# nihalsid/retrieval-fuse

Hardware: AMD Instinct MI355X
Metric: 64^3 TSDF chunks/sec (retrieve+attend+refine) (higher is better)
Workload: dtype f32

## Files before the change

### retrieval-fuse_amd/csrc/build.py

```python
import os
import subprocess
import sys
from concurrent.futures import ThreadPoolExecutor
from pathlib import Path

HERE = Path(__file__).resolve().parent
OUT = HERE.parent / 'rfuse' / 'librfuse_hip.so'
SOURCES = ['capi.hip', 'conv3d.hip', 'conv3d_mfma.hip', 'conv3d_up.hip', 'conv3d_up_split.hip', 'conv3d_split.hip', 'conv3d_split_zc.hip', 'conv3d_e2_split.hip', 'conv3d_small.hip', 'conv3d_backward.hip', 'conv3d_wgrad_split.hip', 'conv_valid_mfma.hip', 'conv_valid_split.hip', 'conv_valid_split_pg.hip', 'conv_valid_backward.hip', 'linear.hip', 'attention.hip', 'attention_backward.hip', 'attention_fused.hip', 'retrieval.hip', 'mesh.hip', 'metrics.hip', 'mesh_metrics.hip', 'shape_loss.hip', 'ntxent.hip', 'iou_matrix.hip']
FLAGS = ['--offload-arch=gfx950', '-O3', '-std=c++17', '-fPIC', '-Wall', '-Wno-unused-function']
EXTRA_FLAGS = {'attention.hip': ['-ffp-contract=off'], 'attention_backward.hip': ['-ffp-contract=off'], 'attention_fused.hip': ['-ffp-contract=off'], 'retrieval.hip': ['-ffp-contract=off'],
               'mesh_metrics.hip': ['-ffp-contract=off'],
               'shape_loss.hip': ['-ffp-contract=off'],
               'ntxent.hip': ['-ffp-contract=off', '-fno-slp-vectorize'],
               'iou_matrix.hip': ['-ffp-contract=off'],
               'conv3d_mfma.hip': ['-fno-slp-vectorize'], 'conv3d_up.hip': ['-fno-slp-vectorize']}


def _hipcc():
    return os.environ.get('HIPCC', '/opt/rocm/bin/hipcc')


def _llvm_bin():
    import shutil
    roots = [Path(os.path.realpath(_hipcc())).parents[1], Path(os.environ.get('ROCM_PATH', '/opt/rocm')), Path('/opt/rocm')]
    for r in roots:
        for sub in ('lib/llvm/bin', 'llvm/bin'):
            if (r / sub / 'llvm-objdump').exists():
                return r / sub
    found = shutil.which('llvm-objdump')
    if found:
        return Path(found).parent
    raise RuntimeError('check_isa: llvm-objdump not found under %s' % ', '.join(str(r) for r in roots))


def _stale(obj, deps):
    return (not obj.exists()) or any(d.stat().st_mtime > obj.stat().st_mtime for d in deps)


def unsafe_packed_fp32(asm_text):
    import re
    bad = []
    for line in asm_text.splitlines():
        m = re.search(r'\bv_pk_(?:fma|mul|add)_f32\b.*?\bop_sel:\[([01,]+)\]', line)
        if m and '1' in m.group(1).split(',')[1:]:
            bad.append(line.strip())
    return bad


def check_isa(so=OUT, name=None):
    import shutil
    import tempfile
    with tempfile.TemporaryDirectory() as tmp:
        lib = Path(tmp) / (name or so.name)
        shutil.copy(so, lib)
        llvm_bin = _llvm_bin()
        subprocess.run([str(llvm_bin / 'llvm-objdump'), '--offloading', str(lib)], check=True, stdout=subprocess.DEVNULL, cwd=tmp)
        cos = sorted(Path(tmp).glob(lib.name + '.*gfx950*'))
        if not cos:
            raise RuntimeError('check_isa: no gfx950 code object found in %s' % so)
        bad = []
        for co in cos:
            asm = subprocess.run([str(llvm_bin / 'llvm-objdump'), '-d', str(co)], check=True, capture_output=True, text=True).stdout
            bad += unsafe_packed_fp32(asm)
    if bad:
        raise RuntimeError('check_isa: %d packed-fp32 instructions with op_sel on src1/src2 (wrong results beside F16 MFMAs on gfx950), e.g.\n  %s'
                           % (len(bad), '\n  '.join(bad[:5])))
    return len(cos)


def build(force=False, verbose=False, out=None, extra_flags=(), objdir=None):
    hipcc = _hipcc()
    OUT = Path(out) if out is not None else globals()['OUT']
    objdir = Path(objdir) if objdir is not None else HERE / 'build'
    objdir.mkdir(exist_ok=True, parents=True)
    headers = [HERE / 'common.h', HERE / 'conv_box.h', HERE / 'conv_split_common.h', HERE / 'conv_split_args.h', HERE / 'split_operand.h', HERE / 'attn_row.h', HERE / 'philox.h',
               HERE.parents[1] / 'include' / 'rfuse.h', HERE.parents[1] / 'include' / 'rfuse_eval.h', HERE.parents[1] / 'include' / 'rfuse_train.h',
               HERE.parents[1] / 'include' / 'rfuse_contrastive.h', HERE.parents[1] / 'include' / 'rfuse_pairs.h', HERE.parents[1] / 'include' / 'rfuse_attn_train.h']

    def compile_one(src):
        obj = objdir / (src.replace('.hip', '.o'))
        if force or _stale(obj, [HERE / src, HERE / 'build.py'] + headers):
            cmd = [hipcc] + FLAGS + list(extra_flags) + EXTRA_FLAGS.get(src, []) + ['-c', str(HERE / src), '-o', str(obj)]
            if verbose:
                print(' '.join(cmd))
            subprocess.run(cmd, check=True)
        return obj

    with ThreadPoolExecutor(max_workers=len(SOURCES)) as ex:
        objs = list(ex.map(compile_one, SOURCES))
    if force or _stale(OUT, objs):
        tmp_out = OUT.with_name(OUT.name + '.unchecked')
        cmd = [hipcc, '--offload-arch=gfx950', '-shared', '-fPIC', '-o', str(tmp_out)] + [str(o) for o in objs]
        if verbose:
            print(' '.join(cmd))
        try:
            subprocess.run(cmd, check=True)
            check_isa(tmp_out, name='librfuse_hip.so')
        except BaseException:
            tmp_out.unlink(missing_ok=True)
            OUT.unlink(missing_ok=True)
            raise
        os.replace(tmp_out, OUT)
    return OUT


TESTKIT_SRC = HERE.parents[1] / 'tests' / 'testkit' / 'testkit.hip'
TESTKIT_OUT = TESTKIT_SRC.parent / 'librfuse_testkit.so'


def build_testkit(force=False):
    if force or _stale(TESTKIT_OUT, [TESTKIT_SRC, HERE / 'build.py']):
        subprocess.run([_hipcc(), '--offload-arch=gfx950', '-O3', '-std=c++17', '-shared', '-fPIC', '-o', str(TESTKIT_OUT), str(TESTKIT_SRC)], check=True)
    return TESTKIT_OUT


if __name__ == '__main__':
    print(build(force='--force' in sys.argv, verbose=True))
    print(build_testkit(force='--force' in sys.argv))
```

### retrieval-fuse_amd/model/unet.py

```python
import math

import torch
from torch import nn

from rfuse import ops, routes


class GroupNormParams(nn.Module):

    def __init__(self, num_groups, num_channels, eps=1e-5):
        super().__init__()
        if num_channels < num_groups:
            num_groups = 1
        assert num_channels % num_groups == 0, \
            f'Expected number of channels in input to be divisible by num_groups. num_channels={num_channels}, num_groups={num_groups}'
        self.num_groups, self.num_channels, self.eps = num_groups, num_channels, eps
        self.weight = nn.Parameter(torch.ones(num_channels))
        self.bias = nn.Parameter(torch.zeros(num_channels))

    def extra_repr(self):
        return f'{self.num_groups}, {self.num_channels}, eps={self.eps}'


class Conv3dParams(nn.Module):
# ... 131 lines not shown
            n, edge, pre = x.n, x.edge, ops.conv3d_split_pre_presplit(x, c1.conv.packed_split(), cmid, *second).data
        else:
            n, ch0, _, edge = ops._src_dims(x, upsampled)
            if route in ('cin1_presplit', 'cin1_presplit_handed'):
                pre = ops.conv3d_cin1_presplit(x, g1.weight, g1.bias, g1.eps, c1.conv.packed(), cmid, *second)
            else:
                aff = ops.gn_affine(x, upsampled, g1.weight, g1.bias, g1.num_groups, g1.eps)
                if route == 'box_presplit':
                    pre = ops.conv3d_split_presplit(x, aff, c1.conv.packed_split(), cmid, *second)
                else:
                    pre = ops.conv3d_up_split_presplit(x, upsampled, aff, c1.conv.packed_up_split(ch0), cmid, *second, parity_major=pm)
        if route == 'cin1_presplit_handed':
            ng = next_block.SingleConv1.groupnorm
            return ops.conv3d_split_pre_relu_pool_presplit(pre, cmid, n, edge, c2.conv.packed_split(), cout, ng.weight, ng.bias, ng.num_groups, ng.eps)
        return ops.conv3d_split_pre_relu(pre, cmid, n, edge, c2.conv.packed_split(), cout, pool=pool, parity_major=pm)


class DoubleConv(_ConvPair):

    def __init__(self, in_channels, out_channels, encoder, kernel_size=3, order='gcr', num_groups=8):
        super().__init__()
        if encoder:
            c1_in, c1_out = in_channels, max(out_channels // 2, in_channels)
            c2_in, c2_out = c1_out, out_channels
        else:
            c1_in, c1_out = in_channels, out_channels
            c2_in, c2_out = out_channels, out_channels
        self.SingleConv1 = SingleConv(c1_in, c1_out, kernel_size, order, num_groups)
        self.SingleConv2 = SingleConv(c2_in, c2_out, kernel_size, order, num_groups)


class StepDownDoubleConv(_ConvPair):
    ENCODER_FORMS = False

    def __init__(self, in_channels, out_channels, encoder, kernel_size=3, order='gcr', num_groups=8):
        super().__init__()
        self.encoder = encoder
        mid = (in_channels + out_channels) // 2
        self.SingleConv1 = SingleConv(in_channels, mid, kernel_size, order, num_groups)
        self.SingleConv2 = SingleConv(mid, out_channels, kernel_size, order, num_groups)


class Encoder(nn.Module):

    def __init__(self, in_channels, out_channels, conv_kernel_size=3, apply_pooling=True, pool_kernel_size=(2, 2, 2),
                 pool_type='max', basic_module=DoubleConv, conv_layer_order='gcr', num_groups=8):
        super().__init__()
        if apply_pooling and (pool_type != 'max' or tuple(pool_kernel_size) != (2, 2, 2)):
            raise NotImplementedError('only MaxPool3d(2) is built')
        self.apply_pooling = apply_pooling
        self.basic_module = basic_module(in_channels, out_channels, encoder=True, kernel_size=conv_kernel_size,
                                         order=conv_layer_order, num_groups=num_groups)

    def forward(self, x, prepooled=None, pool=None, next_block=None):
        if self.apply_pooling:
            if prepooled is not None:
                x = prepooled
            elif ops.needs_grad(x):
                x = torch.nn.functional.max_pool3d(x, 2)
            else:
                x = ops.maxpool2(x)
        return self.basic_module(x, pool=pool, next_block=next_block)


class Decoder(nn.Module):

    def __init__(self, in_channels, out_channels, kernel_size=3, scale_factor=(2, 2, 2), basic_module=DoubleConv,
                 conv_layer_order='gcr', num_groups=8, mode='nearest'):
        super().__init__()
        if basic_module not in (DoubleConv, StepDownDoubleConv) or mode != 'nearest' or tuple(scale_factor) != (2, 2, 2):
            raise NotImplementedError('only nearest x2 upsampling with concat joining is built')
        self.basic_module = basic_module(in_channels, out_channels, encoder=False, kernel_size=kernel_size,
                                         order=conv_layer_order, num_groups=num_groups)

    def forward(self, encoder_features, x):
        if encoder_features.shape[2] != 2 * x.shape[2]:
            raise NotImplementedError('skip connection must be exactly twice the decoder input resolution')
        return self.basic_module(encoder_features, x)


class DecoderNoJoining(Decoder):

    def forward(self, x):
        return self.basic_module(None, x)


def number_of_features_per_level(init_channel_number, num_levels):
    return [init_channel_number * 2 ** k for k in range(num_levels)]


class UNet3D(nn.Module):

    def __init__(self, in_channels, out_channels, final_sigmoid=True, f_maps=64, layer_order='gcr', num_groups=8, num_levels=4,
                 is_segmentation=True, remove_n_final_layers=0, final_conv=False, **kwargs):
        super().__init__()
        if final_conv or is_segmentation:
            raise NotImplementedError('final_conv / segmentation heads are never instantiated by the refinement path')
        if isinstance(f_maps, int):
            f_maps = number_of_features_per_level(f_maps, num_levels=num_levels)
        encoders = []
        for i, out_feature_num in enumerate(f_maps):
            encoders.append(Encoder(in_channels if i == 0 else f_maps[i - 1], out_feature_num, apply_pooling=(i > 0),
                                    basic_module=DoubleConv, conv_layer_order=layer_order, num_groups=num_groups))
        self.encoders = nn.ModuleList(encoders)

        reversed_f_maps = list(reversed(f_maps))
        if remove_n_final_layers > 0:
            reversed_f_maps = reversed_f_maps[:-remove_n_final_layers]
        outs = list(reversed_f_maps)
        outs[-1] = out_channels
        decoders = []
        for i in range(len(reversed_f_maps) - 1):
            in_feature_num = reversed_f_maps[i] + reversed_f_maps[i + 1]
            last_and_trimmed = i == (len(reversed_f_maps) - 2) and remove_n_final_layers > 0
            decoders.append(Decoder(in_feature_num, outs[i + 1], basic_module=StepDownDoubleConv if last_and_trimmed else DoubleConv,
                                    conv_layer_order=layer_order, num_groups=num_groups))
        self.decoders = nn.ModuleList(decoders)

    def forward(self, x, after_encoders=None):
        feats = []
        n_enc, n_dec = len(self.encoders), len(self.decoders)
        pooled = None
        for i, encoder in enumerate(self.encoders):
            if i == n_enc - 1:
                x, pooled = encoder(x, prepooled=pooled), None
            else:
                is_skip = i >= n_enc - 1 - n_dec
                nxt = self.encoders[i + 1].basic_module
                x, pooled = encoder(x, prepooled=pooled, pool='also' if is_skip else 'only', next_block=nxt if isinstance(nxt, DoubleConv) else None)
            feats.insert(0, x)
        feats = feats[1:]
        if after_encoders is not None:
            after_encoders()
        for decoder, skip in zip(self.decoders, feats):
            x = decoder(skip, x)
        return x
```

### retrieval-fuse_amd/rfuse/_lib.py

```python
import ctypes
import os
import re
from pathlib import Path

import torch

_HERE = Path(__file__).resolve().parent
LIB_PATH = Path(os.environ.get('RFUSE_LIB', _HERE / 'librfuse_hip.so'))
HEADER_PATH = _HERE.parents[1] / 'include' / 'rfuse.h'
EVAL_HEADER_PATH = _HERE.parents[1] / 'include' / 'rfuse_eval.h'
TRAIN_HEADER_PATH = _HERE.parents[1] / 'include' / 'rfuse_train.h'
CONTRASTIVE_HEADER_PATH = _HERE.parents[1] / 'include' / 'rfuse_contrastive.h'
PAIRS_HEADER_PATH = _HERE.parents[1] / 'include' / 'rfuse_pairs.h'
ATTN_TRAIN_HEADER_PATH = _HERE.parents[1] / 'include' / 'rfuse_attn_train.h'

_SCALARS = {'int': ctypes.c_int, 'float': ctypes.c_float, 'size_t': ctypes.c_size_t, 'int64_t': ctypes.c_int64, 'long long': ctypes.c_int64}


def parse_header(text):
    text = re.sub(r'/\*.*?\*/', ' ', text, flags=re.S)
    text = re.sub(r'^[ \t]*#.*$', ' ', text, flags=re.M)
    text = re.sub(r'extern\s+"C"\s*\{|\}', ' ', text)

    def where(chunk):
        m = re.search(r'(\w+)\s*\(', chunk)
        return '%s: %r' % (m.group(1) if m else '?', ' '.join(chunk.split()))

    *decls, rest = text.split(';')
    if rest.strip():
        raise ValueError('declaration without its `;` -- %s' % where(rest))

    def ctype(decl, fn, restype=False):
        decl = ' '.join(decl.replace('*', ' * ').split())
        if restype and decl == 'const char *':
            return ctypes.c_char_p
        if decl.endswith('*'):
            return ctypes.c_void_p
        if decl not in _SCALARS:
            raise ValueError('%s: type %r is outside the vocabulary of the binding (%s, pointers)' % (fn, decl, ', '.join(_SCALARS)))
        return _SCALARS[decl]

    table = {}
    for decl in decls:
        m = re.fullmatch(r'\s*([\w\s*]+?)\b(\w+)\s*\(([\w\s*,]*)\)\s*', decl)
        if m is None:
            raise ValueError('cannot read the declaration of %s' % where(decl))
        ret, fn, params = m.groups()
        params = [] if params.strip() == 'void' else [re.fullmatch(r'\s*(\w[\w\s*]*[\s*])(\w+)\s*', q) for q in params.split(',')]
        if None in params:
            raise ValueError('%s: every parameter needs a type and a name' % fn)
        table[fn] = (ctype(ret, fn, True), [ctype(q.group(1), fn) for q in params], [q.group(2) for q in params])
    return table


SIGNATURES = parse_header(HEADER_PATH.read_text())
EVAL_SIGNATURES = parse_header(EVAL_HEADER_PATH.read_text())
TRAIN_SIGNATURES = parse_header(TRAIN_HEADER_PATH.read_text())
CONTRASTIVE_SIGNATURES = parse_header(CONTRASTIVE_HEADER_PATH.read_text())
PAIRS_SIGNATURES = parse_header(PAIRS_HEADER_PATH.read_text())
ATTN_TRAIN_SIGNATURES = parse_header(ATTN_TRAIN_HEADER_PATH.read_text())


def is_status(name, table=None):
    res, _, params = (SIGNATURES if table is None else table)[name]
    return res is ctypes.c_int and params[-1:] == ['stream']


def _raise_on_status(rc, fn, args):
    if rc != 0:
        check(rc, fn.__name__)
    return rc


_lib = None
_eval = None
_train = None
_contrastive = None
_pairs = None
_attn_train = None


class _Library:

    def __init__(self, cdll, table=SIGNATURES):
        self._cdll = cdll
        self._table = table
        self._direct = {}
        for name, (res, args, _) in table.items():
            fn = getattr(cdll, name)
            fn.restype = res
            fn.argtypes = args
            if is_status(name, table):
                fn.errcheck = _raise_on_status
            self._direct[name] = fn
            setattr(self, name, fn)

    def start_profile(self, records, only=None):
        def timed(name, fn):
            def call(*args):
                e0, e1 = torch.cuda.Event(enable_timing=True), torch.cuda.Event(enable_timing=True)
                e0.record()
                rc = fn(*args)
                e1.record()
                records.append((name, tuple(a for a in args if isinstance(a, int)), e0, e1, tuple(i for i, a in enumerate(args) if a is None or (isinstance(a, ctypes.c_void_p) and not a.value))))
                return rc
            return call
        for name, (res, args, _) in self._table.items():
            if only is not None and name not in only:
                continue
            if res is ctypes.c_int and args:
                setattr(self, name, timed(name, self._direct[name]))

    def stop_profile(self):
        for name, fn in self._direct.items():
            setattr(self, name, fn)


def load():
    global _lib
    if _lib is not None:
        return _lib
    if not LIB_PATH.exists():
        raise RuntimeError(
            'librfuse_hip.so not found at %s -- build it with `python retrieval-fuse_amd/csrc/build.py` '
            '(or __graft_entry__.build()).  There is no CPU fallback for the refinement hot path.' % LIB_PATH)
    _lib = _Library(ctypes.CDLL(str(LIB_PATH)))
    return _lib


def load_eval():
    global _eval
    if _eval is None:
        _eval = _Library(load()._cdll, EVAL_SIGNATURES)
    return _eval


def load_train():
    global _train
    if _train is None:
        _train = _Library(load()._cdll, TRAIN_SIGNATURES)
    return _train


def load_contrastive():
    global _contrastive
    if _contrastive is None:
        _contrastive = _Library(load()._cdll, CONTRASTIVE_SIGNATURES)
    return _contrastive


def load_pairs():
    global _pairs
    if _pairs is None:
        _pairs = _Library(load()._cdll, PAIRS_SIGNATURES)
    return _pairs


def load_attn_train():
    global _attn_train
    if _attn_train is None:
        _attn_train = _Library(load()._cdll, ATTN_TRAIN_SIGNATURES)
    return _attn_train


def check(rc, what):
    if rc != 0:
        msg = load().rf_last_error()
        raise RuntimeError('%s failed (rc=%d): %s' % (what, rc, msg.decode() if msg else ''))
```

### retrieval-fuse_amd/rfuse/ops.py

```python
import ctypes
import functools
import sys
import weakref

import torch

from . import _lib

ACT_NONE, ACT_RELU, ACT_LEAKY = 0, 1, 2
ATTN_SOFTMAX, ATTN_GUMBEL_HARD = 0, 1


def _req(t, name, dtype=torch.float32):
    if not isinstance(t, torch.Tensor):
        raise TypeError('%s: expected a torch.Tensor' % name)
    if not t.is_cuda:
        raise RuntimeError('%s: the refinement hot path runs on the GPU only (got a %s tensor); there is no CPU fallback' % (name, t.device))
    if t.dtype != dtype:
        raise TypeError('%s: expected %s, got %s' % (name, dtype, t.dtype))
    if not t.is_contiguous():
        raise ValueError('%s: tensor must be contiguous' % name)
    return t


# ... 85 lines not shown
            st = torch.cuda.current_stream()
            self._event = torch.cuda.Event()
            self._event.record(st)
            self._ok_streams = {st.cuda_stream}

    def wait(self, device, packed=None):
        st = torch.cuda.current_stream(device)
        if st.cuda_stream not in self._ok_streams and not torch.cuda.is_current_stream_capturing():
            st.wait_event(self._event)
            self._ok_streams.add(st.cuda_stream)
            for t in (packed if isinstance(packed, (tuple, list)) else (packed,)):
                if isinstance(t, torch.Tensor):
                    t.record_stream(st)



def _pack_weight(stem, w, dims, dtype=torch.float32, not_taken=None):
    lib = _lib.load()
    if dtype == torch.float32:
        count = getattr(lib, 'rf_%s_packed_floats' % stem)(*dims)
    else:
        count = getattr(lib, 'rf_%s_packed_bytes' % stem)(*dims) // dtype.itemsize
    if count == 0 and not_taken is not None:
        raise ValueError(not_taken)
    out = torch.empty(count, dtype=dtype, device=w.device)
    getattr(lib, 'rf_%s_pack_weight' % stem)(_p(w.detach()), *dims, _p(out), _stream())
    return out


def pack_conv3_weight(w):
    _req(w.detach(), 'conv weight')
    if tuple(w.shape[2:]) != (3, 3, 3):
        raise ValueError('pack_conv3_weight: expected an OIDHW 3x3x3 weight, got %s' % (tuple(w.shape),))
    return _pack_weight('conv3', w, (w.shape[0], w.shape[1]))


def _src_dims(src0, src1):
    n = (src0 if src0 is not None else src1).shape[0]
    c0 = src0.shape[1] if src0 is not None else 0
    c1 = src1.shape[1] if src1 is not None else 0
    edge = src0.shape[2] if src0 is not None else 2 * src1.shape[2]
    for t, e in ((src0, edge), (src1, edge // 2)):
        if t is not None and (t.dim() != 5 or tuple(t.shape[2:]) != (e, e, e) or t.shape[0] != n):
            raise ValueError('expected cubic NCDHW volumes with matching batch, got %s' % (tuple(t.shape),))
    return n, c0, c1, edge


def gn_affine(src0, src1, gamma, beta, groups, eps=1e-5):
    for t, nm in ((src0, 'src0'), (src1, 'src1')):
        if t is not None:
            _req(t, nm)
    _req(gamma.detach(), 'gamma'), _req(beta.detach(), 'beta')
    n, c0, c1, edge = _src_dims(src0, src1)
    c = c0 + c1
    if c < groups:
        groups = 1
    dev = gamma.device
    lib = _lib.load()
    aff = torch.empty((n, c, 4), dtype=torch.float32, device=dev)
    st0, st1 = _fresh_stats(src0), _fresh_stats(src1)
    if (src0 is None or st0 is not None) and (src1 is None or st1 is not None):
        lib.rf_gn_from_stats(_p(st0[0]) if st0 else _p(None), c0, st0[1] if st0 else 0,
                             _p(st1[0]) if st1 else _p(None), c1, st1[1] if st1 else 0, n, edge,
                             _p(gamma.detach()), _p(beta.detach()), groups, eps, _p(aff), _stream())
        return aff
    nbytes = lib.rf_gn_stats_ws_bytes(n, groups)
    ws = _workspace(dev, nbytes)
    lib.rf_gn_stats(_p(src0), c0, _p(src1), c1, n, edge, _p(gamma.detach()), _p(beta.detach()), groups, eps,
                    _p(aff), _p(ws), ws.numel(), _stream())
    return aff


def _check_affine(aff, n, c):
    _req(aff, 'gn affine')
    if tuple(aff.shape) != (n, c, 4):
        raise ValueError('gn affine: expected [%d, %d, 4] (from ops.gn_affine), got %s' % (n, c, tuple(aff.shape)))
    return aff.device


def _attach_stats(t, tiles):
    if t is None:
        return None
    stats = torch.empty((t.shape[0], t.shape[1], tiles, 2), dtype=torch.float64, device=t.device)
    t._rf_stats = (stats, tiles, t._version)
    return stats


def _fresh_stats(t):
    st = getattr(t, '_rf_stats', None) if t is not None else None
    return st if st is not None and st[2] == t._version else None


def _conv_launch(lib, src0, c0, src1, c1, n, edge, aff, w_packed, cout, out):
    tiles = lib.rf_conv3d_stats_tiles(c0, c1, n, edge, cout)
    if tiles > 0:
        lib.rf_conv3d_k3_gn_relu_stats(_p(src0), c0, _p(src1), c1, n, edge, _p(aff), _p(w_packed), cout, _p(out),
                                       _p(_attach_stats(out, tiles)), _stream())
    else:
        lib.rf_conv3d_k3_gn_relu(_p(src0), c0, _p(src1), c1, n, edge, _p(aff), _p(w_packed), cout, _p(out),
                                 _stream())


def conv3d_gn_relu(src0, src1, aff, w_packed, cout, direct_weight=None):
    n, c0, c1, edge = _src_dims(src0, src1)
    dev = _check_affine(aff, n, c0 + c1)
    out = torch.empty((n, cout, edge, edge, edge), dtype=torch.float32, device=dev)
# ... 96 lines not shown
    return w_ok and _abs_max(gamma) * (float(group_elements) ** 0.5) + _abs_max(beta) <= SPLIT_MAX_ABS_ACT


def pack_conv3_split_weight(w):
    _req(w.detach(), 'conv weight')
    if tuple(w.shape[2:]) != (3, 3, 3):
        raise ValueError('pack_conv3_split_weight: expected an OIDHW 3x3x3 weight, got %s' % (tuple(w.shape),))
    return _pack_weight('conv3_split', w, (w.shape[0], w.shape[1]), torch.uint8)


def conv_split_supported(src0, src1, cout):
    if src1 is not None or src0 is None or CONV_ARITH != 'split':
        return False
    n, c0, c1, edge = _src_dims(src0, src1)
    return bool(_lib.load().rf_conv3d_split_supported(c0, c1, n, edge, cout))


def conv3d_split_gn_relu(src, aff, w_split_packed, cout, pool=None):
    n, cin, _, edge = _src_dims(src, None)
    if edge == 4 and pool is not None:
        out = conv3d_split_gn_relu(src, aff, w_split_packed, cout)
        return (out if pool == 'also' else None), maxpool2(out)
    dev = _check_affine(aff, n, cin)
    lib = _lib.load()
    out = torch.empty((n, cout, edge, edge, edge), dtype=torch.float32, device=dev) if pool != 'only' else None
    pooled = torch.empty((n, cout, edge // 2, edge // 2, edge // 2), dtype=torch.float32, device=dev) if pool is not None else None
    tiles = max(1, (edge // 8) ** 3)
    stats, pstats = _attach_stats(out, tiles), _attach_stats(pooled, tiles)
    lib.rf_conv3d_split_k3_gn_relu(_p(src), cin, n, edge, _p(aff), _p(w_split_packed), cout, _p(out), _p(stats), _p(pooled), _p(pstats),
                                   _stream())
    return out if pool is None else (out, pooled)


def pack_conv3_e2_split_weight(w, edge=2):
    _req(w.detach(), 'conv weight')
    if tuple(w.shape[2:]) != (3, 3, 3) or edge not in (1, 2):
        raise ValueError('pack_conv3_e2_split_weight: expected an OIDHW 3x3x3 weight and edge 1 or 2, got %s, edge %r' % (tuple(w.shape), edge))
    return _pack_weight('conv3_e2_split', w, (w.shape[0], w.shape[1], edge), torch.uint8)


def conv_e2_split_supported(src, cout):
    if src is None or CONV_ARITH != 'split':
        return False
    n, c0, _, edge = _src_dims(src, None)
    return bool(_lib.load().rf_conv3d_e2_split_supported(c0, n, edge, cout))


def conv3d_e2_split_gn_relu(src, aff, w_e2_packed, cout):
    n, cin, _, edge = _src_dims(src, None)
    dev = _check_affine(aff, n, cin)
    out = torch.empty((n, cout, edge, edge, edge), dtype=torch.float32, device=dev)
    _lib.load().rf_conv3d_e2_split_k3_gn_relu(_p(src), cin, n, edge, _p(aff), _p(w_e2_packed), cout, _p(out), _p(_attach_stats(out, 1)), _stream())
    return out


USE_PRESPLIT = True


def cin1_presplit_supported(x, cout, next_groups, next_cout):
    if not USE_PRESPLIT or CONV_ARITH != 'split' or x is None or x.shape[1] != 1:
        return False
    n, edge = x.shape[0], x.shape[2]
    lib = _lib.load()
    return bool(lib.rf_conv3d_cin1_presplit_supported(n, edge, cout, next_groups)) and bool(lib.rf_conv3d_split_pre_supported(cout, n, edge, next_cout))


def conv3d_cin1_presplit(x, in_gamma, in_beta, in_eps, w_packed, cout, next_gamma, next_beta, next_groups, eps):
    _req(x, 'x')
    n, edge = x.shape[0], x.shape[2]
    lib = _lib.load()
    out = torch.empty(lib.rf_split_act_bytes(n, cout, edge), dtype=torch.uint8, device=x.device)
    lib.rf_conv3d_cin1_presplit(_p(x), n, edge, _p(in_gamma.detach()), _p(in_beta.detach()), in_eps, _p(w_packed), cout, _p(next_gamma.detach()),
                                _p(next_beta.detach()), next_groups, eps, _p(out), _stream())
    return out


def conv_split_pointwise_supported(x, cout):
    return CONV_ARITH == 'split' and x is not None and bool(_lib.load().rf_conv3d_split_pointwise_supported(x.shape[1], x.shape[0], x.shape[2], cout))


def conv3d_split_pointwise_tanh(x, gn_affine_t, w_split_packed, cout, pw_w, pw_b, post_add=0.0, post_mul=1.0):
    _req(x, 'x')
    n, cin, edge = x.shape[0], x.shape[1], x.shape[2]
    if pw_w.shape[0] != 1:
        raise NotImplementedError('conv3d_split_pointwise_tanh: one output channel (Conv3d(nf,1,1), model/refinement.py:54)')
    out = torch.empty((n, 1, edge, edge, edge), dtype=torch.float32, device=x.device)
    _lib.load().rf_conv3d_split_k3_gn_relu_pointwise_tanh(_p(x), cin, n, edge, _p(gn_affine_t), _p(w_split_packed), cout, _p(pw_w.detach()), _p(pw_b.detach()),
                                                          post_add, post_mul, _p(out), _stream())
    return out


def conv_split_presplit_supported(x, cout, next_groups):
    return (USE_PRESPLIT and CONV_ARITH == 'split' and x is not None
            and bool(_lib.load().rf_conv3d_split_presplit_supported(x.shape[1], x.shape[0], x.shape[2], cout, next_groups)))


def conv3d_split_presplit(x, gn_affine_t, w_split_packed, cout, next_gamma, next_beta, next_groups, eps):
    _req(x, 'x')
    n, cin, edge = x.shape[0], x.shape[1], x.shape[2]
    lib = _lib.load()
    out = torch.empty(lib.rf_split_act_bytes(n, cout, edge), dtype=torch.uint8, device=x.device)
    lib.rf_conv3d_split_presplit(_p(x), cin, n, edge, _p(gn_affine_t), _p(w_split_packed), cout, _p(next_gamma.detach()), _p(next_beta.detach()),
                                 next_groups, eps, _p(out), _p(None), _stream())
    return out


# ... 742 lines not shown
```

### retrieval-fuse_amd/rfuse/routes.py

```python
from . import _lib, ops


def split_arith(range_ok):
    return ops.CONV_ARITH == 'split' and bool(range_ok())


def single(n, c0, c1, edge, cout, pool, split_ok, materialised):
    lib, up, cin = _lib.load(), c1 > 0, c0 + c1
    box = lambda: split_ok and bool(lib.rf_conv3d_split_supported(cin, 0, n, edge, cout))
    e2 = lambda: split_ok and edge <= 2 and bool(lib.rf_conv3d_e2_split_supported(cin, n, edge, cout))
    up_split = lambda: split_ok and up and ops.USE_CONV_UP and bool(lib.rf_conv3d_up_split_supported(c0, c1, n, edge, cout))
    direct = lambda: edge == 1
    if materialised:
        order = (('e2', e2), ('direct', direct), ('split_box', box), ('up_split', up_split))
    else:
        order = (('split_box', lambda: not up and box()),
                 ('e2', lambda: not up and e2()),
                 ('e2_concat', lambda: up and edge == 2 and pool is None and e2()),
                 ('pool_fp32', lambda: pool is not None and not up and edge >= 4 and ops.USE_FUSED_POOL and lib.rf_conv3d_pool_supported(c0, 0, n, edge, cout)),
                 ('direct', direct),
                 ('up_split', up_split),
                 ('split_box_concat', lambda: up and edge >= 8 and box()),
                 ('up_fp32', lambda: up and ops.USE_CONV_UP and lib.rf_conv3d_up_supported(c0, c1, n, edge, cout)))
    return next((name for name, takes in order if takes()), 'generic')


def pair(n, c0, c1, edge, cmid, cout, groups2, pool, grad, range1, range2, offered=False, encoder_forms=True, next_takes=None, next_groups=0):
    if grad or not ops.USE_PRESPLIT or ops.CONV_ARITH != 'split':
        return 'plain'
    lib = _lib.load()
    rest = lambda: lib.rf_conv3d_split_pre_supported(cmid, n, edge, cout) and range1() and range2()
    if offered:
        return 'prepooled' if lib.rf_conv3d_split_pre_presplit_supported(c0, n, edge, cmid, groups2) and rest() else 'plain'
    if c1 == 0 and c0 == 1 and encoder_forms and lib.rf_conv3d_cin1_presplit_supported(n, edge, cmid, groups2) \
            and lib.rf_conv3d_split_pre_supported(cmid, n, edge, cout) and range2():
        if pool == 'only' and next_takes is not None and next_takes() and ops.USE_PREPOOL \
                and lib.rf_conv3d_split_pre_pool_presplit_supported(cmid, n, edge, cout, next_groups):
            return 'cin1_presplit_handed'
        return 'cin1_presplit'
    if c1 > 0 and pool is None and lib.rf_conv3d_up_split_presplit_supported(c0, c1, n, edge, cmid, groups2) and rest():
        pm = c0 > 0 and lib.rf_conv3d_up_split_presplit_pm_supported(c0, c1, n, edge, cmid, groups2) and lib.rf_conv3d_split_pre_pm_supported(cmid, n, edge, cout)
        return 'decoder_presplit_pm' if pm else 'decoder_presplit'
    if c1 == 0 and encoder_forms and lib.rf_conv3d_split_presplit_supported(c0, n, edge, cmid, groups2) and rest():
        return 'box_presplit'
    return 'plain'


def head(n, c1, edge, cmid, cout, range1, range2):
    if ops.CONV_ARITH != 'split':
        return 'plain'
    lib, ok2 = _lib.load(), None
    if ops.USE_CH8 and ops.USE_CONV_UP and lib.rf_conv3d_up_split_ch8_supported(0, c1, n, edge, cmid) \
            and lib.rf_conv3d_split_pointwise_ch8_supported(cmid, n, edge, cout) and range1():
        ok2 = bool(range2())
        if ok2:
            return 'ch8'
    if lib.rf_conv3d_split_pointwise_supported(cmid, n, edge, cout) and (range2() if ok2 is None else ok2):
        return 'pointwise'
    return 'plain'


def _valid_split_takes(lib, n, cin, s, cout, k, stride, range_ok):
    return ops.CONV_ARITH == 'split' and cin % 4 == 0 and range_ok() and bool(lib.rf_conv3d_valid_split_supported(max(n, 1), cin, s, cout, k, stride))


def valid(layer, in_split, nxt=None, fp32_forms=True):
    lib, (n, cin, s, cout, k, stride, range_ok) = _lib.load(), layer
    split = in_split or _valid_split_takes(lib, *layer)
    valu = not split and ops.USE_CONVV_VALU and bool(lib.rf_conv3d_valid_valu_supported(max(n, 1), cin, s, cout, k, stride))
    writes = bool(ops.USE_SPLIT_CHAIN and nxt is not None and cout % 4 == 0 and (split or valu) and _valid_split_takes(lib, *nxt))
    if in_split and writes and ops.USE_CONVV_PG and ops.CONV_ARITH == 'split' \
            and lib.rf_conv3d_valid_split_pg_supported(max(n, 1), cin, s, cout, k, stride) and range_ok():
        return 'grid', True
    if split or valu:
        return ('split' if split else 'valu'), writes
    if not fp32_forms:
        return None, False
    return ('lds' if lib.rf_conv3d_valid_lds_supported(n, cin, s, cout, k, stride) else 'gather'), False


def attn_mlp_fused(n_in, n_out):
    return ops.USE_FUSED_ATTN_MLP and n_in % 16 == 0 and 16 <= n_in <= 128 and n_out == 32
```

Baseline: 5115.

## Fuse deepest encoder level (pool, two GN+conv, decoder GN affine) into one kernel

Adds a single HIP kernel for the bottom 4^3 encoder level. It max-pools the input, applies both GroupNorm+ReLU+conv stages on the 2^3 volume using split-f16 MFMA GEMMs held in LDS, writes the output with its statistics, and optionally precomputes the first decoder's GroupNorm affine from the skip statistics. The Python side routes the last encoder through this kernel, makes the previous encoder skip its pooling output, and caches the ready affine so the decoder can reuse it. The aim is to cut kernel launches and global round-trips at a level where the tensors are tiny. The cost is a 512-thread, one-block-per-CU kernel with heavy LDS use, plus version-tracked caching logic that could go stale.

Result: faster. 5170 (median of 6 runs) (+1.1%).

```diff
diff --git a/include/rfuse_level.h b/include/rfuse_level.h
--- /dev/null
+++ b/include/rfuse_level.h
@@ -0,0 +1,20 @@
+#ifndef RFUSE_LEVEL_H
+#define RFUSE_LEVEL_H
+
+#include <stdint.h>
+#include <stddef.h>
+
+#ifdef __cplusplus
+extern "C" {
+#endif
+
+int rf_conv3d_e2_level_supported(int n, int c, int cmid, int cout, int groups1, int groups2, int c_skip, int tiles_skip, int groups_dec);
+int rf_conv3d_e2_level(const float* x, int n, int c, const float* gamma1, const float* beta1, int groups1, float eps1, const void* w1_packed, int cmid,
+                       const float* gamma2, const float* beta2, int groups2, float eps2, const void* w2_packed, int cout, float* out, double* stats,
+                       const double* skip_stats, int c_skip, int tiles_skip, const float* gamma_dec, const float* beta_dec, int groups_dec,
+                       float eps_dec, float* dec_affine, void* stream);
+
+#ifdef __cplusplus
+}
+#endif
+#endif
diff --git a/retrieval-fuse_amd/csrc/build.py b/retrieval-fuse_amd/csrc/build.py
--- a/retrieval-fuse_amd/csrc/build.py
+++ b/retrieval-fuse_amd/csrc/build.py
@@ -6,7 +6,7 @@
 
 HERE = Path(__file__).resolve().parent
 OUT = HERE.parent / 'rfuse' / 'librfuse_hip.so'
-SOURCES = ['capi.hip', 'conv3d.hip', 'conv3d_mfma.hip', 'conv3d_up.hip', 'conv3d_up_split.hip', 'conv3d_split.hip', 'conv3d_split_zc.hip', 'conv3d_e2_split.hip', 'conv3d_small.hip', 'conv3d_backward.hip', 'conv3d_wgrad_split.hip', 'conv_valid_mfma.hip', 'conv_valid_split.hip', 'conv_valid_split_pg.hip', 'conv_valid_backward.hip', 'linear.hip', 'attention.hip', 'attention_backward.hip', 'attention_fused.hip', 'retrieval.hip', 'mesh.hip', 'metrics.hip', 'mesh_metrics.hip', 'shape_loss.hip', 'ntxent.hip', 'iou_matrix.hip']
+SOURCES = ['capi.hip', 'conv3d.hip', 'conv3d_mfma.hip', 'conv3d_up.hip', 'conv3d_up_split.hip', 'conv3d_split.hip', 'conv3d_split_zc.hip', 'conv3d_e2_split.hip', 'conv3d_e2_level.hip', 'conv3d_small.hip', 'conv3d_backward.hip', 'conv3d_wgrad_split.hip', 'conv_valid_mfma.hip', 'conv_valid_split.hip', 'conv_valid_split_pg.hip', 'conv_valid_backward.hip', 'linear.hip', 'attention.hip', 'attention_backward.hip', 'attention_fused.hip', 'retrieval.hip', 'mesh.hip', 'metrics.hip', 'mesh_metrics.hip', 'shape_loss.hip', 'ntxent.hip', 'iou_matrix.hip']
 FLAGS = ['--offload-arch=gfx950', '-O3', '-std=c++17', '-fPIC', '-Wall', '-Wno-unused-function']
 EXTRA_FLAGS = {'attention.hip': ['-ffp-contract=off'], 'attention_backward.hip': ['-ffp-contract=off'], 'attention_fused.hip': ['-ffp-contract=off'], 'retrieval.hip': ['-ffp-contract=off'],
                'mesh_metrics.hip': ['-ffp-contract=off'],
@@ -75,7 +75,8 @@
     objdir.mkdir(exist_ok=True, parents=True)
     headers = [HERE / 'common.h', HERE / 'conv_box.h', HERE / 'conv_split_common.h', HERE / 'conv_split_args.h', HERE / 'split_operand.h', HERE / 'attn_row.h', HERE / 'philox.h',
                HERE.parents[1] / 'include' / 'rfuse.h', HERE.parents[1] / 'include' / 'rfuse_eval.h', HERE.parents[1] / 'include' / 'rfuse_train.h',
-               HERE.parents[1] / 'include' / 'rfuse_contrastive.h', HERE.parents[1] / 'include' / 'rfuse_pairs.h', HERE.parents[1] / 'include' / 'rfuse_attn_train.h']
+               HERE.parents[1] / 'include' / 'rfuse_contrastive.h', HERE.parents[1] / 'include' / 'rfuse_pairs.h', HERE.parents[1] / 'include' / 'rfuse_attn_train.h',
+               HERE.parents[1] / 'include' / 'rfuse_level.h']
 
     def compile_one(src):
         obj = objdir / (src.replace('.hip', '.o'))
diff --git a/retrieval-fuse_amd/csrc/conv3d_e2_level.hip b/retrieval-fuse_amd/csrc/conv3d_e2_level.hip
--- /dev/null
+++ b/retrieval-fuse_amd/csrc/conv3d_e2_level.hip
@@ -0,0 +1,307 @@
+#include "common.h"
+#include "split_operand.h"
+#include "../../include/rfuse_level.h"
+
+namespace {
+constexpr int LV_M = 32;
+constexpr int LV_THREADS = 512;
+constexpr int LV_NC = 256;
+constexpr int LV_STEP_H8 = (LV_NC / 16) * 2 * 64;
+constexpr int LV_CMAX = 64;
+constexpr int LV_COMAX = 128;
+constexpr int LV_A_BYTES = (LV_CMAX / 4) * 2 * 2 * 64 * 16;
+constexpr int LV_S_BYTES = LV_M * LV_COMAX * 16;
+constexpr int LV_LDS_BYTES = LV_A_BYTES + LV_S_BYTES;
+constexpr int LV_RING = 3;
+static_assert(LV_M * LV_CMAX * 16 * 2 <= LV_S_BYTES, "statistics and triples of a 64-channel tensor share the S region");
+}
+
+struct LvArgs {
+    const float* x;
+    float* out;
+    double2* stats;
+    const h8 *w1, *w2;
+    const float *g1, *b1, *g2, *b2;
+    const double2* skip_stats;
+    const float *gd, *bd;
+    float4* dec;
+    double eps1, eps2, epsd;
+    int n, c, cm, co, groups1, groups2, c_skip, t_skip, groups_d;
+};
+
+template <int D>
+__device__ __forceinline__ int lv_xor32(int v) {
+    static_assert(D == 1 || D == 2 || D == 4, "inside 8 lanes");
+    if constexpr (D == 1) return __builtin_amdgcn_update_dpp(0, v, 0xB1, 0xf, 0xf, false);
+    else if constexpr (D == 2) return __builtin_amdgcn_update_dpp(0, v, 0x4E, 0xf, 0xf, false);
+    else {
+        const int t = __builtin_amdgcn_update_dpp(0, v, 0x104, 0xf, 0x5, false);
+        return __builtin_amdgcn_update_dpp(t, v, 0x114, 0xf, 0xA, false);
+    }
+}
+template <int D>
+__device__ __forceinline__ double lv_xor(double x) {
+    return __hiloint2double(lv_xor32<D>(__double2hiint(x)), lv_xor32<D>(__double2loint(x)));
+}
+
+__device__ __forceinline__ void lv_seq_sum(const double2* p, int len, double& sm, double& sq) {
+    for (int i0 = 0; i0 < len; i0 += 8) {
+        double2 v[8];
+#pragma unroll
+        for (int k = 0; k < 8; ++k) v[k] = p[i0 + k < len ? i0 + k : len - 1];
+#pragma unroll
+        for (int k = 0; k < 8; ++k)
+            if (i0 + k < len) { sm += v[k].x; sq += v[k].y; }
+    }
+}
+
+__device__ __forceinline__ void lv_gemm(const h8* __restrict__ aimg, const h8* __restrict__ wb, int ks, int lane, f32x4 (&hi)[2][4], f32x4 (&lo)[2][4]) {
+    h8 ring[LV_RING][8];
+    auto load = [&](int slot, int s) {
+#pragma unroll
+        for (int q = 0; q < 8; ++q) ring[slot][q] = wb[(size_t)s * LV_STEP_H8 + q * 64];
+    };
+#pragma unroll
+    for (int i = 0; i < 2; ++i)
+#pragma unroll
+        for (int j = 0; j < 4; ++j) { hi[i][j] = f32x4{0.f, 0.f, 0.f, 0.f}; lo[i][j] = f32x4{0.f, 0.f, 0.f, 0.f}; }
+#pragma unroll
+    for (int r = 0; r < LV_RING - 1; ++r) load(r, r);
+#pragma unroll
+    for (int s = 0; s < LV_CMAX / 4; ++s) {
+        {
+            const int r = s % LV_RING;
+            if (s >= ks) break;
+            if (s + LV_RING - 1 < ks) load((r + LV_RING - 1) % LV_RING, s + LV_RING - 1);
+            h8 ah[2], al[2];
+#pragma unroll
+            for (int i = 0; i < 2; ++i) {
+                ah[i] = aimg[((s * 2 + i) * 2 + 0) * 64 + lane];
+                al[i] = aimg[((s * 2 + i) * 2 + 1) * 64 + lane];
+            }
+#pragma unroll
+            for (int j = 0; j < 4; ++j)
+#pragma unroll
+                for (int i = 0; i < 2; ++i) hi[i][j] = __builtin_amdgcn_mfma_f32_16x16x32_f16(ah[i], ring[r][2 * j], hi[i][j], 0, 0, 0);
+#pragma unroll
+            for (int j = 0; j < 4; ++j)
+#pragma unroll
+                for (int i = 0; i < 2; ++i) lo[i][j] = __builtin_amdgcn_mfma_f32_16x16x32_f16(ah[i], ring[r][2 * j + 1], lo[i][j], 0, 0, 0);
+#pragma unroll
+            for (int j = 0; j < 4; ++j)
+#pragma unroll
+                for (int i = 0; i < 2; ++i) lo[i][j] = __builtin_amdgcn_mfma_f32_16x16x32_f16(al[i], ring[r][2 * j], lo[i][j], 0, 0, 0);
+        }
+    }
+}
+
+__device__ __forceinline__ void lv_triples(const double2* st, float4* trip, int C, int cpg, double count, double eps, const float* __restrict__ gamma,
+                                           const float* __restrict__ beta, int tid) {
+    for (int u = tid; u < LV_M * C; u += LV_THREADS) {
+        const int sl = u / C, c = u - sl * C, ca = (c / cpg) * cpg;
+        const double2* p = st + sl * C + ca;
+        double sm = 0.0, sq = 0.0;
+        lv_seq_sum(p, cpg, sm, sq);
+        trip[u] = rf_gn_triple(sm, sq, count, eps, gamma[c], beta[c]);
+    }
+}
+
+__global__ __launch_bounds__(LV_THREADS, 1) void k_conv3_e2_level(LvArgs a) {
+    extern __shared__ __attribute__((aligned(16))) unsigned char lds_raw[];
+    h8* aimg = reinterpret_cast<h8*>(lds_raw);
+    _Float16* a16 = reinterpret_cast<_Float16*>(lds_raw);
+    double2* st = reinterpret_cast<double2*>(lds_raw + LV_A_BYTES);
+    float4* trip = reinterpret_cast<float4*>(lds_raw + LV_A_BYTES + LV_S_BYTES / 2);
+    const int tid = threadIdx.x, lane = tid & 63;
+    const int wave = __builtin_amdgcn_readfirstlane(tid >> 6);
+    const int li = lane & 15, kg = lane >> 4;
+    const int n0 = blockIdx.x * LV_M;
+    const int C = a.c, CM = a.cm, CO = a.co;
+
+    const int planes = LV_M * C;
+    const int o = tid & 7, ox = o & 1, oy = (o >> 1) & 1, oz = o >> 2;
+    const int voff = ((2 * oz) * 4 + 2 * oy) * 4 + 2 * ox;
+    float m[32];
+#pragma unroll
+    for (int b = 0; b < 4; ++b) {
+        float2 v[8][4];
+#pragma unroll
+        for (int q = 0; q < 8; ++q) {
+            const int pl = (b * 8 + q) * 64 + (tid >> 3);
+            const int sl = pl / C;
+            const bool live = pl < planes && n0 + sl < a.n;
+            const float* src = a.x + ((size_t)n0 * C + (live ? pl : 0)) * 64 + voff;
+#pragma unroll
+            for (int d = 0; d < 4; ++d) v[q][d] = *reinterpret_cast<const float2*>(src + ((d >> 1) * 4 + (d & 1)) * 4);
+        }
+#pragma unroll
+        for (int q = 0; q < 8; ++q) {
+            const int pl = (b * 8 + q) * 64 + (tid >> 3);
+            const int sl = pl / C;
+            const bool live = pl < planes && n0 + sl < a.n;
+            float mm = -INFINITY;
+#pragma unroll
+            for (int d = 0; d < 4; ++d) mm = rf_max(mm, rf_max(v[q][d].x, v[q][d].y));
+            mm = live ? mm : 0.f;
+            m[b * 8 + q] = mm;
+            double sm = (double)mm, sq = (double)mm * mm;
+            sm += lv_xor<4>(sm); sq += lv_xor<4>(sq);
+            sm += lv_xor<2>(sm); sq += lv_xor<2>(sq);
+            sm += lv_xor<1>(sm); sq += lv_xor<1>(sq);
+            if (o == 0 && pl < planes) st[pl] = make_double2(sm, sq);
+        }
+    }
+    __syncthreads();
+    lv_triples(st, trip, C, C / a.groups1, (double)(C / a.groups1) * 8.0, a.eps1, a.g1, a.b1, tid);
+    __syncthreads();
+#pragma unroll
+    for (int it = 0; it < 32; ++it) {
+        const int pl = it * 64 + (tid >> 3);
+        if (pl < planes) {
+            const int sl = pl / C, c = pl - sl * C;
+            const float4 t = trip[pl];
+            _Float16 h, l;
+            rf_split(fmaf(m[it] - t.x, t.y, t.z) * SPLIT_ACT_SCALE, h, l);
+            const int e = ((((c >> 2) * 2 + (sl >> 4)) * 2) * 64 + (c & 3) * 16 + (sl & 15)) * 8 + o;
+            a16[e] = h;
+            a16[e + 64 * 8] = l;
+        }
+    }
+    __syncthreads();
+
+    f32x4 hi[2][4], lo[2][4];
+    const int ks1 = C >> 2, ks2 = CM >> 2, t0 = (wave & 3) * 4;
+    lv_gemm(aimg, a.w1 + ((size_t)(wave >> 2) * ks1) * LV_STEP_H8 + t0 * 128 + lane, ks1, lane, hi, lo);
+#pragma unroll
+    for (int i = 0; i < 2; ++i)
+#pragma unroll
+        for (int j = 0; j < 4; ++j)
+#pragma unroll
+            for (int r = 0; r < 4; ++r) {
+                const float y = rf_relu(rf_split_join(hi[i][j][r], lo[i][j][r]));
+                hi[i][j][r] = y;
+                double sv = (double)y, sq = (double)y * (double)y;
+                sv += lv_xor<1>(sv); sq += lv_xor<1>(sq);
+                sv += lv_xor<2>(sv); sq += lv_xor<2>(sq);
+                sv += lv_xor<4>(sv); sq += lv_xor<4>(sq);
+                if ((li & 7) == 0) st[(i * 16 + kg * 4 + r) * CM + wave * 8 + j * 2 + (li >> 3)] = make_double2(sv, sq);
+            }
+    __syncthreads();
+    lv_triples(st, trip, CM, CM / a.groups2, (double)(CM / a.groups2) * 8.0, a.eps2, a.g2, a.b2, tid);
+    __syncthreads();
+#pragma unroll
+    for (int i = 0; i < 2; ++i)
+#pragma unroll
+        for (int j = 0; j < 4; ++j) {
+            const int cm = wave * 8 + j * 2 + (li >> 3);
+#pragma unroll
+            for (int r = 0; r < 4; ++r) {
+                const int row = kg * 4 + r;
+                const float4 t = trip[(i * 16 + row) * CM + cm];
+                _Float16 h, l;
+                rf_split(fmaf(hi[i][j][r] - t.x, t.y, t.z) * SPLIT_ACT_SCALE, h, l);
+                const int e = ((((cm >> 2) * 2 + i) * 2) * 64 + (cm & 3) * 16 + row) * 8 + (li & 7);
+                a16[e] = h;
+                a16[e + 64 * 8] = l;
+            }
+        }
+    __syncthreads();
+
+    const int ncols = CO * 8;
+    const bool table = a.dec != nullptr;
+    for (int pass = 0; pass < ncols / 512; ++pass) {
+        lv_gemm(aimg, a.w2 + ((size_t)(pass * 2 + (wave >> 2)) * ks2) * LV_STEP_H8 + t0 * 128 + lane, ks2, lane, hi, lo);
+#pragma unroll
+        for (int i = 0; i < 2; ++i)
+#pragma unroll
+            for (int j = 0; j < 4; ++j) {
+                const int col = pass * 512 + wave * 64 + j * 16 + li;
+#pragma unroll
+                for (int r = 0; r < 4; ++r) {
+                    const int row = i * 16 + kg * 4 + r, sm = n0 + row;
+                    const float y = rf_relu(rf_split_join(hi[i][j][r], lo[i][j][r]));
+                    const bool live = sm < a.n;
+                    if (live) a.out[(size_t)sm * ncols + col] = y;
+                    double sv = (double)y, sq = (double)y * (double)y;
+                    sv += lv_xor<1>(sv); sq += lv_xor<1>(sq);
+                    sv += lv_xor<2>(sv); sq += lv_xor<2>(sq);
+                    sv += lv_xor<4>(sv); sq += lv_xor<4>(sq);
+                    if ((li & 7) == 0) {
+                        if (live) a.stats[(size_t)sm * CO + (col >> 3)] = make_double2(sv, sq);
+                        if (table) st[row * CO + (col >> 3)] = make_double2(sv, sq);
+                    }
+                }
+            }
+    }
+    if (!table) return;
+
+    __syncthreads();
+    double2* gs = reinterpret_cast<double2*>(lds_raw);
+    const int c0 = a.c_skip, CD = c0 + CO, GD = a.groups_d, cpg = CD / GD, tl = a.t_skip;
+    for (int u = tid; u < LV_M * GD; u += LV_THREADS) {
+        const int sl = u / GD, g = u - sl * GD, nn = n0 + sl;
+        if (nn >= a.n) continue;
+        const int ca = g * cpg, cb = ca + cpg;
+        double sm = 0.0, sq = 0.0;
+        {
+            const int hi_c = cb < c0 ? cb : c0;
+            if (ca < hi_c) {
+                const double2* p = a.skip_stats + ((size_t)nn * c0 + ca) * tl;
+                const int len = (hi_c - ca) * tl;
+                lv_seq_sum(p, len, sm, sq);
+            }
+        }
+        {
+            const int lo_c = ca > c0 ? ca : c0;
+            if (lo_c < cb) {
+                const double2* p = st + sl * CO + (lo_c - c0);
+                const int len = cb - lo_c;
+                double s1 = 0.0, s2 = 0.0;
+                lv_seq_sum(p, len, s1, s2);
+                sm += 8.0 * s1;
+                sq += 8.0 * s2;
+            }
+        }
+        gs[u] = make_double2(sm, sq);
+    }
+    __syncthreads();
+    const double count = (double)cpg * 64.0;
+    for (int e = tid; e < LV_M * CD; e += LV_THREADS) {
+        const int sl = e / CD, c = e - sl * CD, nn = n0 + sl;
+        if (nn >= a.n) continue;
+        const double2 s = gs[sl * GD + c / cpg];
+        a.dec[(size_t)nn * CD + c] = rf_gn_triple(s.x, s.y, count, a.epsd, a.gd[c], a.bd[c]);
+    }
+}
+
+static bool lv_gn_plan(int n, int channels, int groups, int tiles) {
+    return groups > 0 && channels % groups == 0 && (long long)n * groups >= 1024 && (long long)(channels / groups) * tiles <= 128;
+}
+
+extern "C" int rf_conv3d_e2_level_supported(int n, int c, int cmid, int cout, int groups1, int groups2, int c_skip, int tiles_skip, int groups_dec) {
+    if (n < 1 || c < 8 || c > LV_CMAX || c % 4 != 0 || cmid != 64 || (cout != 64 && cout != LV_COMAX)) return 0;
+    if (!lv_gn_plan(n, c, groups1, 1) || !lv_gn_plan(n, cmid, groups2, 1)) return 0;
+    if (c_skip < 0 || (c_skip > 0 && (tiles_skip < 1 || groups_dec > 128 || !lv_gn_plan(n, c_skip + cout, groups_dec, tiles_skip)))) return 0;
+    return 1;
+}
+
+extern "C" int rf_conv3d_e2_level(const float* x, int n, int c, const float* gamma1, const float* beta1, int groups1, float eps1, const void* w1_packed, int cmid,
+                                  const float* gamma2, const float* beta2, int groups2, float eps2, const void* w2_packed, int cout, float* out, double* stats,
+                                  const double* skip_stats, int c_skip, int tiles_skip, const float* gamma_dec, const float* beta_dec, int groups_dec,
+                                  float eps_dec, float* dec_affine, void* stream) {
+    RF_REQUIRE(rf_conv3d_e2_level_supported(n, c, cmid, cout, groups1, groups2, c_skip, tiles_skip, groups_dec), RF_E_UNSUPPORTED,
+               "rf_conv3d_e2_level: takes c = 8 .. 64 (a multiple of 4), cmid 64, cout 64 or 128, and GroupNorm plans of at least 1024 (sample, group) units with at most "
+               "128 entries per group (got n=%d c=%d cmid=%d cout=%d groups=%d,%d skip=%d x %d tiles, %d groups)", n, c, cmid, cout, groups1, groups2, c_skip,
+               tiles_skip, groups_dec);
+    RF_REQUIRE(x && gamma1 && beta1 && w1_packed && gamma2 && beta2 && w2_packed && out && stats, RF_E_INVALID, "rf_conv3d_e2_level: null pointer");
+    RF_REQUIRE(c_skip == 0 || (skip_stats && gamma_dec && beta_dec && dec_affine), RF_E_INVALID, "rf_conv3d_e2_level: null pointer (decoder table)");
+    LvArgs a;
+    a.x = x; a.out = out; a.stats = reinterpret_cast<double2*>(stats);
+    a.w1 = reinterpret_cast<const h8*>(w1_packed); a.w2 = reinterpret_cast<const h8*>(w2_packed);
+    a.g1 = gamma1; a.b1 = beta1; a.g2 = gamma2; a.b2 = beta2;
+    a.skip_stats = c_skip ? reinterpret_cast<const double2*>(skip_stats) : nullptr;
+    a.gd = gamma_dec; a.bd = beta_dec; a.dec = c_skip ? reinterpret_cast<float4*>(dec_affine) : nullptr;
+    a.eps1 = (double)eps1; a.eps2 = (double)eps2; a.epsd = (double)eps_dec;
+    a.n = n; a.c = c; a.cm = cmid; a.co = cout; a.groups1 = groups1; a.groups2 = groups2; a.c_skip = c_skip; a.t_skip = tiles_skip; a.groups_d = groups_dec;
+    return rf_launch<k_conv3_e2_level>("rf_conv3d_e2_level", dim3((unsigned)((n + LV_M - 1) / LV_M)), dim3(LV_THREADS), LV_LDS_BYTES, LV_LDS_BYTES, (hipStream_t)stream, a);
+}
diff --git a/retrieval-fuse_amd/model/unet.py b/retrieval-fuse_amd/model/unet.py
--- a/retrieval-fuse_amd/model/unet.py
+++ b/retrieval-fuse_amd/model/unet.py
@@ -207,15 +207,45 @@
         self.basic_module = basic_module(in_channels, out_channels, encoder=True, kernel_size=conv_kernel_size,
                                          order=conv_layer_order, num_groups=num_groups)
 
-    def forward(self, x, prepooled=None, pool=None, next_block=None):
+    def level_route(self, n, c, edge, grad=False, skip=None):
+        bm = self.basic_module
+        if not self.apply_pooling or not isinstance(bm, DoubleConv) or bm.SingleConv1.conv.in_channels != c:
+            return 'plain'
+        c1, c2 = bm.SingleConv1, bm.SingleConv2
+        grad = grad or (torch.is_grad_enabled() and any(p.requires_grad for p in self.parameters()))
+        return routes.level(n, c, edge, c1.conv.out_channels, c2.conv.out_channels, ops._gn_groups(c, c1.groupnorm.num_groups),
+                            ops._gn_groups(c1.conv.out_channels, c2.groupnorm.num_groups), grad, c1.range_ok(edge // 2), c2.range_ok(edge // 2), skip=skip)
+
+    def forward(self, x, prepooled=None, pool=None, next_block=None, consumer=None):
         if self.apply_pooling:
             if prepooled is not None:
                 x = prepooled
             elif ops.needs_grad(x):
                 x = torch.nn.functional.max_pool3d(x, 2)
             else:
+                if pool is None and x.dim() == 5:
+                    done = self._whole_level(x, consumer)
+                    if done is not None:
+                        return done
                 x = ops.maxpool2(x)
         return self.basic_module(x, pool=pool, next_block=next_block)
+
+    def _whole_level(self, x, consumer):
+        n, c, edge = x.shape[0], x.shape[1], x.shape[2]
+        skip = gn_dec = None
+        if consumer is not None and consumer[0] is not None:
+            st = ops._fresh_stats(consumer[0])
+            if st is not None:
+                skip, gn_dec = consumer
+        cout = self.basic_module.SingleConv2.conv.out_channels if isinstance(self.basic_module, DoubleConv) else 0
+        plan = None if skip is None else (skip.shape[1], st[1], ops._gn_groups(skip.shape[1] + cout, gn_dec.num_groups))
+        if self.level_route(n, c, edge, skip=plan) != 'e2_level':
+            return None
+        c1, c2 = self.basic_module.SingleConv1, self.basic_module.SingleConv2
+        g1, g2 = c1.groupnorm, c2.groupnorm
+        return ops.conv3d_e2_level(x, (g1.weight, g1.bias, g1.num_groups, g1.eps), c1.conv.packed_e2_split(2), c1.conv.out_channels,
+                                   (g2.weight, g2.bias, g2.num_groups, g2.eps), c2.conv.packed_e2_split(2), cout, skip=skip,
+                                   gn_dec=None if skip is None else (gn_dec.weight, gn_dec.bias, gn_dec.num_groups, gn_dec.eps))
 
 
 class Decoder(nn.Module):
@@ -278,11 +308,19 @@
         pooled = None
         for i, encoder in enumerate(self.encoders):
             if i == n_enc - 1:
-                x, pooled = encoder(x, prepooled=pooled), None
+                consumer = (feats[0], self.decoders[0].basic_module.SingleConv1.groupnorm) if n_dec > 0 and feats and isinstance(self.decoders[0], Decoder) \
+                    and not isinstance(self.decoders[0], DecoderNoJoining) else None
+                x, pooled = encoder(x, prepooled=pooled, consumer=consumer), None
             else:
                 is_skip = i >= n_enc - 1 - n_dec
                 nxt = self.encoders[i + 1].basic_module
-                x, pooled = encoder(x, prepooled=pooled, pool='also' if is_skip else 'only', next_block=nxt if isinstance(nxt, DoubleConv) else None)
+                cout = encoder.basic_module.SingleConv2.conv.out_channels
+                src = pooled if pooled is not None else x
+                n, edge = (src.n, src.edge) if isinstance(src, ops.PreSplit) else (src.shape[0], src.shape[2])
+                if i == n_enc - 2 and is_skip and self.encoders[i + 1].level_route(n, cout, edge, ops.needs_grad(x)) == 'e2_level':
+                    x, pooled = encoder(x, prepooled=pooled, next_block=nxt if isinstance(nxt, DoubleConv) else None), None
+                else:
+                    x, pooled = encoder(x, prepooled=pooled, pool='also' if is_skip else 'only', next_block=nxt if isinstance(nxt, DoubleConv) else None)
             feats.insert(0, x)
         feats = feats[1:]
         if after_encoders is not None:
diff --git a/retrieval-fuse_amd/rfuse/_lib.py b/retrieval-fuse_amd/rfuse/_lib.py
--- a/retrieval-fuse_amd/rfuse/_lib.py
+++ b/retrieval-fuse_amd/rfuse/_lib.py
@@ -13,6 +13,7 @@
 CONTRASTIVE_HEADER_PATH = _HERE.parents[1] / 'include' / 'rfuse_contrastive.h'
 PAIRS_HEADER_PATH = _HERE.parents[1] / 'include' / 'rfuse_pairs.h'
 ATTN_TRAIN_HEADER_PATH = _HERE.parents[1] / 'include' / 'rfuse_attn_train.h'
+LEVEL_HEADER_PATH = _HERE.parents[1] / 'include' / 'rfuse_level.h'
 
 _SCALARS = {'int': ctypes.c_int, 'float': ctypes.c_float, 'size_t': ctypes.c_size_t, 'int64_t': ctypes.c_int64, 'long long': ctypes.c_int64}
 
@@ -59,6 +60,7 @@
 CONTRASTIVE_SIGNATURES = parse_header(CONTRASTIVE_HEADER_PATH.read_text())
 PAIRS_SIGNATURES = parse_header(PAIRS_HEADER_PATH.read_text())
 ATTN_TRAIN_SIGNATURES = parse_header(ATTN_TRAIN_HEADER_PATH.read_text())
+LEVEL_SIGNATURES = parse_header(LEVEL_HEADER_PATH.read_text())
 
 
 def is_status(name, table=None):
@@ -78,6 +80,7 @@
 _contrastive = None
 _pairs = None
 _attn_train = None
+_level = None
 
 
 class _Library:
@@ -163,6 +166,13 @@
     return _attn_train
 
 
+def load_level():
+    global _level
+    if _level is None:
+        _level = _Library(load()._cdll, LEVEL_SIGNATURES)
+    return _level
+
+
 def check(rc, what):
     if rc != 0:
         msg = load().rf_last_error()
diff --git a/retrieval-fuse_amd/rfuse/ops.py b/retrieval-fuse_amd/rfuse/ops.py
--- a/retrieval-fuse_amd/rfuse/ops.py
+++ b/retrieval-fuse_amd/rfuse/ops.py
@@ -161,6 +161,9 @@
             _req(t, nm)
     _req(gamma.detach(), 'gamma'), _req(beta.detach(), 'beta')
     n, c0, c1, edge = _src_dims(src0, src1)
+    ready = _ready_affine(src0, src1, gamma, beta, groups, eps)
+    if ready is not None:
+        return ready
     c = c0 + c1
     if c < groups:
         groups = 1
@@ -363,6 +366,49 @@
     out = torch.empty((n, cout, edge, edge, edge), dtype=torch.float32, device=dev)
     _lib.load().rf_conv3d_e2_split_k3_gn_relu(_p(src), cin, n, edge, _p(aff), _p(w_e2_packed), cout, _p(out), _p(_attach_stats(out, 1)), _stream())
     return out
+
+
+USE_E2_LEVEL = True
+
+
+def _gn_groups(c, groups):
+    return 1 if c < groups else groups
+
+
+def conv3d_e2_level(x, gn1, w1_e2_packed, cmid, gn2, w2_e2_packed, cout, skip=None, gn_dec=None):
+    _req(x, 'x')
+    n, c, _, edge = _src_dims(x, None)
+    if edge != 4:
+        raise ValueError('conv3d_e2_level: expected 4^3 volumes, got %s' % (tuple(x.shape),))
+    for g in (gn1, gn2) + ((gn_dec,) if skip is not None else ()):
+        _req(g[0].detach(), 'gamma'), _req(g[1].detach(), 'beta')
+    lib = _lib.load_level()
+    out = torch.empty((n, cout, 2, 2, 2), dtype=torch.float32, device=x.device)
+    stats = _attach_stats(out, 1)
+    st0 = aff = None
+    if skip is not None:
+        st0, c_skip = _fresh_stats(skip), skip.shape[1]
+        if st0 is None or tuple(skip.shape) != (n, c_skip, 4, 4, 4):
+            raise ValueError('conv3d_e2_level: the skip tensor must be [n, c_skip, 4,4,4] and carry its producer\'s statistics')
+        aff = torch.empty((n, c_skip + cout, 4), dtype=torch.float32, device=x.device)
+    lib.rf_conv3d_e2_level(_p(x), n, c, _p(gn1[0].detach()), _p(gn1[1].detach()), _gn_groups(c, gn1[2]), gn1[3], _p(w1_e2_packed), cmid,
+                           _p(gn2[0].detach()), _p(gn2[1].detach()), _gn_groups(cmid, gn2[2]), gn2[3], _p(w2_e2_packed), cout, _p(out), _p(stats),
+                           _p(st0[0]) if st0 else _p(None), skip.shape[1] if st0 else 0, st0[1] if st0 else 0,
+                           _p(gn_dec[0].detach()) if st0 else _p(None), _p(gn_dec[1].detach()) if st0 else _p(None),
+                           _gn_groups(skip.shape[1] + cout, gn_dec[2]) if st0 else 0, gn_dec[3] if st0 else 0.0, _p(aff), _stream())
+    if aff is not None:
+        out._rf_ready_affine = (aff, out._version, weakref.ref(skip), skip._version, weakref.ref(gn_dec[0]), gn_dec[0]._version,
+                                weakref.ref(gn_dec[1]), gn_dec[1]._version, gn_dec[2], gn_dec[3])
+    return out
+
+
+def _ready_affine(src0, src1, gamma, beta, groups, eps):
+    r = getattr(src1, '_rf_ready_affine', None) if src0 is not None and src1 is not None else None
+    if r is None:
+        return None
+    aff, v1, ref0, v0, refg, vg, refb, vb, g, e = r
+    same = ref0() is src0 and refg() is gamma and refb() is beta
+    return aff if same and (v1, v0, vg, vb, g, e) == (src1._version, src0._version, gamma._version, beta._version, groups, eps) else None
 
 
 USE_PRESPLIT = True
diff --git a/retrieval-fuse_amd/rfuse/routes.py b/retrieval-fuse_amd/rfuse/routes.py
--- a/retrieval-fuse_amd/rfuse/routes.py
+++ b/retrieval-fuse_amd/rfuse/routes.py
@@ -46,6 +46,20 @@
     return 'plain'
 
 
+def level(n, c, edge, cmid, cout, groups1, groups2, grad, range1, range2, skip=None):
+    if grad or not ops.USE_E2_LEVEL or ops.CONV_ARITH != 'split' or edge != 4:
+        return 'plain'
+    c_skip, tiles, groups_dec = skip if skip is not None else (0, 0, 0)
+    if not _lib.load_level().rf_conv3d_e2_level_supported(n, c, cmid, cout, groups1, groups2, c_skip, tiles, groups_dec):
+        return 'plain'
+    ok1 = bool(range1())
+    ok2 = ok1 and bool(range2())
+    if not ok2 or pair(n, c, 0, 2, cmid, cout, groups2, None, False, lambda: ok1, lambda: ok2) != 'plain':
+        return 'plain'
+    both_e2 = single(n, c, 0, 2, cmid, None, True, False) == 'e2' and single(n, cmid, 0, 2, cout, None, True, False) == 'e2'
+    return 'e2_level' if both_e2 else 'plain'
+
+
 def head(n, c1, edge, cmid, cout, range1, range2):
     if ops.CONV_ARITH != 'split':
         return 'plain'
```
